# facebookresearch/PoseDiffusion

Measured on AMD Instinct MI355X. Metric: sequences/sec (20-frame, GGS on), higher is better.
Workload: dtype f32 (GGS, attention, LayerNorm, DDPM update, every accumulation); the encoder GEMMs multiply fp16 hi + lo operand pairs (22 bits, static power-of-two scales) with fp32 accumulation -- `exact_mode` is the same pipe with them on the exact-fp32 matrix instruction

## Files before the change

### posediffusion_amd/csrc/pd_qkv_attn.h

```cpp
#pragma once
#include "pd_gemm_split.h"

#ifndef PD_QA_XCD_MAP
#define PD_QA_XCD_MAP 1
#endif
#define PD_QA_WAVES 12
#define PD_QA_THREADS (PD_QA_WAVES * 64)
#define PD_QA_ROWS 96
#define PD_QA_LDR (3 * DH + 4)
#define PD_QA_LS 36
#ifndef PD_QA_DEEP_DEFAULT
#define PD_QA_DEEP_DEFAULT 0
#endif

struct PdQkvAttnArgs {
    const unsigned *A;
    const unsigned *W;
    const float *bias;
    unsigned *ctx;
    int B, N, G;
    float c_scale, out_scale;
};
static inline int pd_qkv_attn_group(int N) { return N >= 1 && N <= 32 ? (PD_QA_ROWS - 1) / N : 0; }
static inline int pd_qkv_attn_wgs(int B, int N) {
    const int G = pd_qkv_attn_group(N);
    return G ? ((B + G - 1) / G) * NH : 0;
}
static inline size_t pd_qkv_attn_lds(int N) {
    const int G = pd_qkv_attn_group(N);
    const size_t image = (size_t)(G * N + 1) * PD_QA_LDR * sizeof(float);
    const size_t stage = (size_t)4 * PD_QA_ROWS * 32 * sizeof(unsigned);
    return (image > stage ? image : stage) + (size_t)3 * 32 * PD_QA_LS * sizeof(float);
}

template <int BARE, bool DEEP = false>
__global__ __launch_bounds__(PD_QA_THREADS) void pd_qkv_attn_kernel(PdQkvAttnArgs g) {
    constexpr int KC = 32, RT = 3, TM = PD_QA_ROWS, CHA = TM * KC, LDR = PD_QA_LDR, LS = PD_QA_LS;
    constexpr bool M16 = PD_STRIP_MFMA16 != 0;
    extern __shared__ __attribute__((aligned(1024))) unsigned qa_lds[];
    const int tid = threadIdx.x, lane = tid & 63, l31 = lane & 31, hi = lane >> 5;
    const int wave = __builtin_amdgcn_readfirstlane(tid >> 6);
    int head = blockIdx.x & 3, grp = blockIdx.x >> 2;
#if PD_QA_XCD_MAP == 1
    {
        const int ngrp = gridDim.x >> 2, c = blockIdx.x >> 4, r = blockIdx.x & 15;
        if (4 * c + 4 <= ngrp) {
            head = 2 * ((r & 7) >> 2) + (r >> 3);
            grp = 4 * c + (r & 3);
        }
    }
#elif PD_QA_XCD_MAP == 2
    {
        const int ngrp = gridDim.x >> 2, c = blockIdx.x >> 5, r = blockIdx.x & 31;
        if (8 * c + 8 <= ngrp) {
            head = r >> 3;
            grp = 8 * c + (r & 7);
        }
    }
#endif
    const int N = g.N, G = g.G, M = g.B * N;
    const int seq0 = grp * G, nseq = min(G, g.B - seq0), m0 = seq0 * N, rows = nseq * N;
    const int nt16 = __builtin_amdgcn_readfirstlane((rows + 15) >> 4);
    const int stages = __builtin_amdgcn_readfirstlane(8 * wave < 16 * nt16 ? 1 : 0);
    const int prow = lane >> 3, pslot = lane & 7, l15 = lane & 15, kg = lane >> 4;
    unsigned oa;
    {
        const int r = 8 * wave + prow;
        oa = (unsigned)(((size_t)min(m0 + r, M - 1) * DM + 4 * (pslot ^ pd_strip_swz<M16>(r))) * sizeof(unsigned));
    }
    const unsigned lds_a = (unsigned)(size_t)(qa_lds + wave * 256);
    const int third = wave >> 2;
    const int ntile = third * (DM / 32) + head * (DH / 32) + (wave & 3);
    constexpr int KS = DM / 16;
    const uint4 *wq = (const uint4 *)g.W + (size_t)ntile * KS * 128 + (M16 ? (kg >> 1) * 128 + (kg & 1) * 32 + l15 : lane);
    typedef unsigned wv4 __attribute__((ext_vector_type(4)));
    f32x16 acc[M16 ? 1 : RT];
    f32x4 acc4[M16 ? 2 * RT : 1][2];
#pragma unroll
    for (int mi = 0; mi < (M16 ? 1 : RT); ++mi)
#pragma unroll
        for (int i = 0; i < 16; ++i) acc[mi][i] = 0.0f;
#pragma unroll
    for (int t = 0; t < (M16 ? 2 * RT : 1); ++t) acc4[t][0] = acc4[t][1] = f32x4{0.f, 0.f, 0.f, 0.f};
    auto mmaw = [](const uint4 &a, const wv4 &b, const f32x16 &c) {
        return __builtin_amdgcn_mfma_f32_32x32x16_f16(__builtin_bit_cast(f16x8, a), __builtin_bit_cast(f16x8, b), c, 0, 0, 0);
    };
    auto mma16 = [](const uint4 &a, const wv4 &b, const f32x4 &c) {
        return __builtin_amdgcn_mfma_f32_16x16x32_f16(__builtin_bit_cast(f16x8, a), __builtin_bit_cast(f16x8, b), c, 0, 0, 0);
    };
#define PD_QA_WLOAD(w0, w1, w2, w3, b)                                                                                               \
    do {                                                                                                                             \
        const uint4 *wp_ = wq + (size_t)(b) * 256;                                                                                   \
        if constexpr (M16)                                                                                                           \
            asm volatile("global_load_dwordx4 %0, %4, off\n\tglobal_load_dwordx4 %1, %4, off offset:1024\n\t"                       \
                         "global_load_dwordx4 %2, %4, off offset:256\n\tglobal_load_dwordx4 %3, %4, off offset:1280"                 \
                         : "=&v"(w0), "=&v"(w1), "=&v"(w2), "=&v"(w3) : "v"(wp_) : "memory");                                        \
        else                                                                                                                         \
            asm volatile("global_load_dwordx4 %0, %4, off\n\tglobal_load_dwordx4 %1, %4, off offset:1024\n\t"                       \
                         "global_load_dwordx4 %2, %4, off offset:2048\n\tglobal_load_dwordx4 %3, %4, off offset:3072"                \
                         : "=&v"(w0), "=&v"(w1), "=&v"(w2), "=&v"(w3) : "v"(wp_) : "memory");                                        \
    } while (0)
#define PD_QA_WAIT(n, w0, w1, w2, w3) asm volatile("s_waitcnt vmcnt(" #n ")" : "+v"(w0), "+v"(w1), "+v"(w2), "+v"(w3) : : "memory")
#define PD_QA_WAIT_STAGED(stg, w0, w1, w2, w3)                                                                                       \
    asm volatile("s_cmp_eq_u32 %4, 0\n\ts_cbranch_scc1 .Lqa_ns%=\n\ts_waitcnt vmcnt(6)\n\ts_branch .Lqa_done%=\n"                   \
                 ".Lqa_ns%=:\n\ts_waitcnt vmcnt(4)\n.Lqa_done%=:"                                                                   \
                 : "+v"(w0), "+v"(w1), "+v"(w2), "+v"(w3) : "s"(__builtin_amdgcn_readfirstlane(stg)) : "memory", "scc")
    auto stage64 = [&](int c, int buf) {
        if (!stages) return;
        const unsigned da = __builtin_amdgcn_readfirstlane(lds_a + buf * 2 * CHA * 4);
#pragma unroll
        for (int h = 0; h < 2; ++h) pd_dma_piece((const float *)(g.A + (2 * c + h) * KC), oa, da + h * CHA * 4);
    };
    auto block = [&](auto nt_, const unsigned *a, const wv4 &w0, const wv4 &w1, const wv4 &w2, const wv4 &w3) {
        constexpr int NT = decltype(nt_)::value;
        if constexpr (M16) {
            const int sz = pd_strip_swz<true>(l15);
#pragma unroll
            for (int t = 0; t < NT; ++t) {
                const uint4 p = *(const uint4 *)(a + t * 16 * KC + 4 * ((2 * kg) ^ sz));
                const uint4 q = *(const uint4 *)(a + t * 16 * KC + 4 * ((2 * kg + 1) ^ sz));
                const uint4 h8 = make_uint4(__builtin_amdgcn_perm(p.y, p.x, 0x05040100u), __builtin_amdgcn_perm(p.w, p.z, 0x05040100u),
                                            __builtin_amdgcn_perm(q.y, q.x, 0x05040100u), __builtin_amdgcn_perm(q.w, q.z, 0x05040100u));
                const uint4 l8 = make_uint4(__builtin_amdgcn_perm(p.y, p.x, 0x07060302u), __builtin_amdgcn_perm(p.w, p.z, 0x07060302u),
                                            __builtin_amdgcn_perm(q.y, q.x, 0x07060302u), __builtin_amdgcn_perm(q.w, q.z, 0x07060302u));
                f32x4 &c0 = acc4[M16 ? t : 0][0], &c1 = acc4[M16 ? t : 0][1];
                c0 = mma16(l8, w0, c0); c1 = mma16(l8, w2, c1);
                c0 = mma16(h8, w1, c0); c1 = mma16(h8, w3, c1);
                c0 = mma16(h8, w0, c0); c1 = mma16(h8, w2, c1);
            }
        } else {
        uint4 ah[RT], al[RT];
#pragma unroll
        for (int st = 0; st < 2; ++st) {
#pragma unroll
            for (int mi = 0; mi < RT; ++mi) {
                const uint4 p = *(const uint4 *)(a + mi * 32 * KC + 4 * ((4 * st + 2 * hi) ^ ((l31 >> 1) & 7)));
                const uint4 q = *(const uint4 *)(a + mi * 32 * KC + 4 * ((4 * st + 2 * hi + 1) ^ ((l31 >> 1) & 7)));
                ah[mi] = make_uint4(__builtin_amdgcn_perm(p.y, p.x, 0x05040100u), __builtin_amdgcn_perm(p.w, p.z, 0x05040100u),
                                    __builtin_amdgcn_perm(q.y, q.x, 0x05040100u), __builtin_amdgcn_perm(q.w, q.z, 0x05040100u));
                al[mi] = make_uint4(__builtin_amdgcn_perm(p.y, p.x, 0x07060302u), __builtin_amdgcn_perm(p.w, p.z, 0x07060302u),
                                    __builtin_amdgcn_perm(q.y, q.x, 0x07060302u), __builtin_amdgcn_perm(q.w, q.z, 0x07060302u));
            }
            const wv4 &wh = st ? w2 : w0, &wl = st ? w3 : w1;
#pragma unroll
            for (int mi = 0; mi < RT; ++mi) acc[M16 ? 0 : mi] = mmaw(al[mi], wh, acc[M16 ? 0 : mi]);
#pragma unroll
            for (int mi = 0; mi < RT; ++mi) acc[M16 ? 0 : mi] = mmaw(ah[mi], wl, acc[M16 ? 0 : mi]);
#pragma unroll
            for (int mi = 0; mi < RT; ++mi) acc[M16 ? 0 : mi] = mmaw(ah[mi], wh, acc[M16 ? 0 : mi]);
        }
        }
    };
    const int lrow = M16 ? l15 : l31;
    auto kloop = [&](auto nt_) {
        wv4 a0, a1, a2, a3, b0, b1, b2, b3;
        constexpr int nk64 = DM / 64;
        stage64(0, 0);
        PD_QA_WLOAD(a0, a1, a2, a3, 0);
        PD_QA_WLOAD(b0, b1, b2, b3, 1);
        PD_QA_WAIT(0, a0, a1, a2, a3);
        PD_QA_WAIT(0, b0, b1, b2, b3);
        __syncthreads();
        if constexpr (DEEP) {
            static_assert(!DEEP || BARE == 0, "the deep form has no development variants");
            wv4 c0, c1, c2, c3, d0, d1, d2, d3;
            for (int c = 0; c < nk64; c += 2) {
                {
                    const unsigned *a = qa_lds + 0 * 2 * CHA + lrow * KC;
                    stage64(c + 1, 1);
                    PD_QA_WLOAD(c0, c1, c2, c3, 2 * (c + 1));
                    PD_QA_WLOAD(d0, d1, d2, d3, 2 * (c + 1) + 1);
                    block(nt_, a, a0, a1, a2, a3);
                    block(nt_, a + CHA, b0, b1, b2, b3);
                    PD_QA_WAIT(0, c0, c1, c2, c3);
                    PD_QA_WAIT(0, d0, d1, d2, d3);
                    __syncthreads();
                }
                {
                    const int cn = min(c + 2, nk64 - 1);
                    const unsigned *a = qa_lds + 1 * 2 * CHA + lrow * KC;
                    stage64(cn, 0);
                    PD_QA_WLOAD(a0, a1, a2, a3, 2 * cn);
                    PD_QA_WLOAD(b0, b1, b2, b3, 2 * cn + 1);
                    block(nt_, a, c0, c1, c2, c3);
                    block(nt_, a + CHA, d0, d1, d2, d3);
                    PD_QA_WAIT(0, a0, a1, a2, a3);
                    PD_QA_WAIT(0, b0, b1, b2, b3);
                    __syncthreads();
                }
            }
        } else
        for (int c = 0; c < nk64; ++c) {
            const int cn = min(c + 1, nk64 - 1);
            const unsigned *a = qa_lds + (c & 1) * 2 * CHA + lrow * KC;
            if constexpr (BARE == 0) {
                if (c + 1 < nk64) {
                    stage64(cn, (c + 1) & 1);
                    block(nt_, a, a0, a1, a2, a3);
                    PD_QA_WLOAD(a0, a1, a2, a3, 2 * cn);
                    PD_QA_WAIT_STAGED(stages, b0, b1, b2, b3);
                    block(nt_, a + CHA, b0, b1, b2, b3);
                    PD_QA_WLOAD(b0, b1, b2, b3, 2 * cn + 1);
                    PD_QA_WAIT(4, a0, a1, a2, a3);
                } else {
                    block(nt_, a, a0, a1, a2, a3);
                    PD_QA_WAIT(0, b0, b1, b2, b3);
                    block(nt_, a + CHA, b0, b1, b2, b3);
                }
            } else {
                if constexpr (BARE != 2 && BARE != 3) stage64(cn, (c + 1) & 1);
                if constexpr (BARE != 4) block(nt_, a, a0, a1, a2, a3);
                if constexpr (BARE != 1 && BARE != 3) PD_QA_WLOAD(a0, a1, a2, a3, 2 * cn);
                if constexpr (BARE != 4) block(nt_, a + CHA, b0, b1, b2, b3);
                if constexpr (BARE != 1 && BARE != 3) PD_QA_WLOAD(b0, b1, b2, b3, 2 * cn + 1);
                PD_QA_WAIT(0, a0, a1, a2, a3);
                PD_QA_WAIT(0, b0, b1, b2, b3);
            }
            __syncthreads();
        }
        PD_QA_WAIT(0, b0, b1, b2, b3);
    };
    if constexpr (M16) {
        switch (nt16) {
        case 1: kloop(std::integral_constant<int, 1>()); break;
        case 2: kloop(std::integral_constant<int, 2>()); break;
        case 3: kloop(std::integral_constant<int, 3>()); break;
        case 4: kloop(std::integral_constant<int, 4>()); break;
        case 5: kloop(std::integral_constant<int, 5>()); break;
        default: kloop(std::integral_constant<int, 6>()); break;
        }
    } else {
        kloop(std::integral_constant<int, 6>());
    }
#undef PD_QA_WLOAD
#undef PD_QA_WAIT
#undef PD_QA_WAIT_STAGED
    if constexpr (BARE == 5) {
        if (acc[0][0] + acc4[0][0][0] == 123.456f) g.ctx[tid] = 1u;
        return;
    }
    float *img = (float *)qa_lds;
    float *Sall = img + (size_t)(G * N + 1) * LDR;
    {
        const float qscale = 0.08838834764831845f;
        if constexpr (M16) {
#pragma unroll
            for (int ct = 0; ct < 2; ++ct) {
                const float bias = g.bias[ntile * 32 + 16 * ct + l15];
                const int lcol = third * DH + (wave & 3) * 32 + 16 * ct + l15;
#pragma unroll
                for (int t = 0; t < 2 * RT; ++t)
#pragma unroll
                    for (int i = 0; i < 4; ++i) {
                        const int row = 16 * t + 4 * kg + i;
                        float v = fmaf(acc4[M16 ? t : 0][ct][i], g.c_scale, bias);
                        if (third == 0) v *= qscale;
                        if (row < rows) img[row * LDR + lcol] = v;
                    }
            }
        } else {
        const int col = ntile * 32 + l31;
        const float bias = g.bias[col];
        const int lcol = third * DH + (wave & 3) * 32 + l31;
#pragma unroll
        for (int mi = 0; mi < RT; ++mi)
#pragma unroll
            for (int i = 0; i < 16; ++i) {
                const int row = mi * 32 + 4 * hi + (i & 3) + 8 * (i >> 2);
                float v = fmaf(acc[M16 ? 0 : mi][i], g.c_scale, bias);
                if (third == 0) v *= qscale;
                if (row < rows) img[row * LDR + lcol] = v;
            }
        }
        for (int c = tid; c < LDR; c += PD_QA_THREADS) img[G * N * LDR + c] = 0.0f;
    }
    __syncthreads();
    const int team = wave >> 2, tw = wave & 3, ttid = tid & 255;
    float *S = Sall + team * 32 * LS;
    const int rounds = (G + 2) / 3;
    for (int rd = 0; rd < rounds; ++rd) {
        const int s = rd * 3 + team;
        const bool active = s < nseq;
        const float *base = img + (size_t)s * N * LDR;
        const float *zrow = img + (size_t)G * N * LDR;
        auto rowp = [&](int j) { return j < N ? base + j * LDR : zrow; };
        if (active) {
            const float *qa = rowp(16 * (tw >> 1) + (lane & 15)) + 4 * (lane >> 4);
            const float *kb = rowp(16 * (tw & 1) + (lane & 15)) + DH + 4 * (lane >> 4);
            f32x4 sc = {0.f, 0.f, 0.f, 0.f};
#pragma unroll
            for (int c = 0; c < DH / 16; ++c) {
                const float4 a = *(const float4 *)(qa + 16 * c), k = *(const float4 *)(kb + 16 * c);
                sc = __builtin_amdgcn_mfma_f32_16x16x4f32(a.x, k.x, sc, 0, 0, 0);
                sc = __builtin_amdgcn_mfma_f32_16x16x4f32(a.y, k.y, sc, 0, 0, 0);
                sc = __builtin_amdgcn_mfma_f32_16x16x4f32(a.z, k.z, sc, 0, 0, 0);
                sc = __builtin_amdgcn_mfma_f32_16x16x4f32(a.w, k.w, sc, 0, 0, 0);
            }
            const int j = 16 * (tw & 1) + (lane & 15);
#pragma unroll
            for (int e = 0; e < 4; ++e) S[(16 * (tw >> 1) + 4 * (lane >> 4) + e) * LS + j] = sc[e];
        }
        __syncthreads();
        if (active) {
            const int i = ttid >> 3, sub = ttid & 7;
            float4 sv = *(const float4 *)(S + i * LS + 4 * sub);
            const int j0 = 4 * sub;
            sv.x = j0 + 0 < N ? sv.x : -INFINITY;
            sv.y = j0 + 1 < N ? sv.y : -INFINITY;
            sv.z = j0 + 2 < N ? sv.z : -INFINITY;
            sv.w = j0 + 3 < N ? sv.w : -INFINITY;
            float mx = fmaxf(fmaxf(sv.x, sv.y), fmaxf(sv.z, sv.w));
            mx = fmaxf(mx, __shfl_xor(mx, 1, 64));
            mx = fmaxf(mx, __shfl_xor(mx, 2, 64));
            mx = fmaxf(mx, __shfl_xor(mx, 4, 64));
            float4 e;
            e.x = j0 + 0 < N ? expf(sv.x - mx) : 0.0f;
            e.y = j0 + 1 < N ? expf(sv.y - mx) : 0.0f;
            e.z = j0 + 2 < N ? expf(sv.z - mx) : 0.0f;
            e.w = j0 + 3 < N ? expf(sv.w - mx) : 0.0f;
            const float inv = 1.0f / pd_sum8((e.x + e.y) + (e.z + e.w));
            e.x *= inv; e.y *= inv; e.z *= inv; e.w *= inv;
            *(float4 *)(S + i * LS + 4 * sub) = e;
        }
        __syncthreads();
        if (active) {
            f32x4 o[2][2];
#pragma unroll
            for (int rt = 0; rt < 2; ++rt)
#pragma unroll
                for (int ct = 0; ct < 2; ++ct) o[rt][ct] = f32x4{0.f, 0.f, 0.f, 0.f};
            const float *pa = S + (lane & 15) * LS + 4 * (lane >> 4);
            const int vcol = 2 * DH + 32 * tw + (lane & 15);
            const int jg = 4 * (lane >> 4);
#pragma unroll
            for (int c = 0; c < 2; ++c) {
                const float4 p0 = *(const float4 *)(pa + 16 * c), p1 = *(const float4 *)(pa + 16 * LS + 16 * c);
                float v0[4], v1[4];
#pragma unroll
                for (int e = 0; e < 4; ++e) {
                    const float *vr = rowp(16 * c + jg + e) + vcol;
                    v0[e] = vr[0];
                    v1[e] = vr[16];
                }
                const float a0[4] = {p0.x, p0.y, p0.z, p0.w}, a1[4] = {p1.x, p1.y, p1.z, p1.w};
#pragma unroll
                for (int e = 0; e < 4; ++e) {
                    o[0][0] = __builtin_amdgcn_mfma_f32_16x16x4f32(a0[e], v0[e], o[0][0], 0, 0, 0);
                    o[0][1] = __builtin_amdgcn_mfma_f32_16x16x4f32(a0[e], v1[e], o[0][1], 0, 0, 0);
                    o[1][0] = __builtin_amdgcn_mfma_f32_16x16x4f32(a1[e], v0[e], o[1][0], 0, 0, 0);
                    o[1][1] = __builtin_amdgcn_mfma_f32_16x16x4f32(a1[e], v1[e], o[1][1], 0, 0, 0);
                }
            }
#pragma unroll
            for (int rt = 0; rt < 2; ++rt)
#pragma unroll
                for (int e = 0; e < 4; ++e) {
                    const int i = 16 * rt + 4 * (lane >> 4) + e;
                    if (i < N) {
                        unsigned *out = g.ctx + (size_t)((seq0 + s) * N + i) * DM + head * DH + 32 * tw + (lane & 15);
#pragma unroll
                        for (int ct = 0; ct < 2; ++ct) out[16 * ct] = pd_split_word_as<2>(o[rt][ct][e], g.out_scale);
                    }
                }
        }
        __syncthreads();
    }
}

static inline void pd_qkv_attn(const unsigned *hn, const unsigned *Wh, const float *bias, unsigned *ctx, int B, int N, float c_scale, float out_scale,
                               hipStream_t s) {
    PdQkvAttnArgs g{hn, Wh, bias, ctx, B, N, pd_qkv_attn_group(N), c_scale, out_scale};
    const dim3 grid(pd_qkv_attn_wgs(B, N)), blk(PD_QA_THREADS);
    const size_t lds = pd_qkv_attn_lds(N);
#ifdef PD_DEV_KNOBS
    static const int bare = pd_dev_knob("PD_QA_BARE", 0);
    static const int deep = pd_dev_knob("PD_QA_DEEP", PD_QA_DEEP_DEFAULT);
    if (bare == 0 && !deep) { hipLaunchKernelGGL((pd_qkv_attn_kernel<0, false>), grid, blk, lds, s, g); return; }
    switch (bare) {
    case 1: hipLaunchKernelGGL(pd_qkv_attn_kernel<1>, grid, blk, lds, s, g); return;
    case 2: hipLaunchKernelGGL(pd_qkv_attn_kernel<2>, grid, blk, lds, s, g); return;
    case 3: hipLaunchKernelGGL(pd_qkv_attn_kernel<3>, grid, blk, lds, s, g); return;
    case 4: hipLaunchKernelGGL(pd_qkv_attn_kernel<4>, grid, blk, lds, s, g); return;
    case 5: hipLaunchKernelGGL(pd_qkv_attn_kernel<5>, grid, blk, lds, s, g); return;
    default: break;
    }
#endif
    hipLaunchKernelGGL((pd_qkv_attn_kernel<0, PD_QA_DEEP_DEFAULT != 0>), grid, blk, lds, s, g);
}
```

Baseline: 1105.

## Give each wave its own attention row tile and replace block barriers with wave syncs

The attention phase of the fused QKV+attention kernel no longer runs in rounds of three 4-wave teams separated by block-wide barriers. Each wave now owns one (sequence, 16-row) unit. It computes the scores for all 32 keys, does the softmax, and does the full 128-wide PV product, using only wavefront fences and barriers. The score scratch grows to hold every sequence's rows at once. Dropping the __syncthreads rounds should remove barrier stalls, but with 20 frames some of the 12 waves sit idle, and each wave carries more accumulators, which raises register pressure.

```diff
diff --git a/posediffusion_amd/csrc/pd_qkv_attn.h b/posediffusion_amd/csrc/pd_qkv_attn.h
--- a/posediffusion_amd/csrc/pd_qkv_attn.h
+++ b/posediffusion_amd/csrc/pd_qkv_attn.h
@@ -30,7 +30,7 @@
     const int G = pd_qkv_attn_group(N);
     const size_t image = (size_t)(G * N + 1) * PD_QA_LDR * sizeof(float);
     const size_t stage = (size_t)4 * PD_QA_ROWS * 32 * sizeof(unsigned);
-    return (image > stage ? image : stage) + (size_t)3 * 32 * PD_QA_LS * sizeof(float);
+    return (image > stage ? image : stage) + (size_t)PD_QA_ROWS * PD_QA_LS * sizeof(float);
 }
 
 template <int BARE, bool DEEP = false>
@@ -275,35 +275,48 @@
         for (int c = tid; c < LDR; c += PD_QA_THREADS) img[G * N * LDR + c] = 0.0f;
     }
     __syncthreads();
-    const int team = wave >> 2, tw = wave & 3, ttid = tid & 255;
-    float *S = Sall + team * 32 * LS;
-    const int rounds = (G + 2) / 3;
-    for (int rd = 0; rd < rounds; ++rd) {
-        const int s = rd * 3 + team;
-        const bool active = s < nseq;
+    float *S = Sall;
+    const float *zrow = img + (size_t)G * N * LDR;
+    const int nrt = (N + 15) >> 4, units = nseq * nrt;
+    auto wave_sync = [] {
+        __builtin_amdgcn_fence(__ATOMIC_SEQ_CST, "wavefront");
+        __builtin_amdgcn_wave_barrier();
+    };
+    for (int u = wave; u < units; u += PD_QA_WAVES) {
+        const int s = nrt == 2 ? u >> 1 : u, rt = nrt == 2 ? u & 1 : 0;
         const float *base = img + (size_t)s * N * LDR;
-        const float *zrow = img + (size_t)G * N * LDR;
         auto rowp = [&](int j) { return j < N ? base + j * LDR : zrow; };
-        if (active) {
-            const float *qa = rowp(16 * (tw >> 1) + (lane & 15)) + 4 * (lane >> 4);
-            const float *kb = rowp(16 * (tw & 1) + (lane & 15)) + DH + 4 * (lane >> 4);
-            f32x4 sc = {0.f, 0.f, 0.f, 0.f};
+        float *St = S + (size_t)(s * N + 16 * rt) * LS;
+        {
+            const float *qa = rowp(16 * rt + l15) + 4 * kg;
+            const float *kb0 = rowp(l15) + DH + 4 * kg, *kb1 = rowp(16 + l15) + DH + 4 * kg;
+            f32x4 sc0 = {0.f, 0.f, 0.f, 0.f}, sc1 = {0.f, 0.f, 0.f, 0.f};
 #pragma unroll
             for (int c = 0; c < DH / 16; ++c) {
-                const float4 a = *(const float4 *)(qa + 16 * c), k = *(const float4 *)(kb + 16 * c);
-                sc = __builtin_amdgcn_mfma_f32_16x16x4f32(a.x, k.x, sc, 0, 0, 0);
-                sc = __builtin_amdgcn_mfma_f32_16x16x4f32(a.y, k.y, sc, 0, 0, 0);
-                sc = __builtin_amdgcn_mfma_f32_16x16x4f32(a.z, k.z, sc, 0, 0, 0);
-                sc = __builtin_amdgcn_mfma_f32_16x16x4f32(a.w, k.w, sc, 0, 0, 0);
-            }
-            const int j = 16 * (tw & 1) + (lane & 15);
-#pragma unroll
-            for (int e = 0; e < 4; ++e) S[(16 * (tw >> 1) + 4 * (lane >> 4) + e) * LS + j] = sc[e];
-        }
-        __syncthreads();
-        if (active) {
-            const int i = ttid >> 3, sub = ttid & 7;
-            float4 sv = *(const float4 *)(S + i * LS + 4 * sub);
+                const float4 a = *(const float4 *)(qa + 16 * c), k0 = *(const float4 *)(kb0 + 16 * c), k1 = *(const float4 *)(kb1 + 16 * c);
+                sc0 = __builtin_amdgcn_mfma_f32_16x16x4f32(a.x, k0.x, sc0, 0, 0, 0);
+                sc1 = __builtin_amdgcn_mfma_f32_16x16x4f32(a.x, k1.x, sc1, 0, 0, 0);
+                sc0 = __builtin_amdgcn_mfma_f32_16x16x4f32(a.y, k0.y, sc0, 0, 0, 0);
+                sc1 = __builtin_amdgcn_mfma_f32_16x16x4f32(a.y, k1.y, sc1, 0, 0, 0);
+                sc0 = __builtin_amdgcn_mfma_f32_16x16x4f32(a.z, k0.z, sc0, 0, 0, 0);
+                sc1 = __builtin_amdgcn_mfma_f32_16x16x4f32(a.z, k1.z, sc1, 0, 0, 0);
+                sc0 = __builtin_amdgcn_mfma_f32_16x16x4f32(a.w, k0.w, sc0, 0, 0, 0);
+                sc1 = __builtin_amdgcn_mfma_f32_16x16x4f32(a.w, k1.w, sc1, 0, 0, 0);
+            }
+#pragma unroll
+            for (int e = 0; e < 4; ++e)
+                if (16 * rt + 4 * kg + e < N) {
+                    St[(4 * kg + e) * LS + l15] = sc0[e];
+                    St[(4 * kg + e) * LS + 16 + l15] = sc1[e];
+                }
+        }
+        wave_sync();
+#pragma unroll
+        for (int p = 0; p < 2; ++p) {
+            const int i = 8 * p + (lane >> 3), sub = lane & 7;
+            const bool live = 16 * rt + i < N;
+            float *sp = St + (live ? i : N - 1 - 16 * rt) * LS + 4 * sub;
+            float4 sv = *(const float4 *)sp;
             const int j0 = 4 * sub;
             sv.x = j0 + 0 < N ? sv.x : -INFINITY;
             sv.y = j0 + 1 < N ? sv.y : -INFINITY;
@@ -320,50 +333,40 @@
             e.w = j0 + 3 < N ? expf(sv.w - mx) : 0.0f;
             const float inv = 1.0f / pd_sum8((e.x + e.y) + (e.z + e.w));
             e.x *= inv; e.y *= inv; e.z *= inv; e.w *= inv;
-            *(float4 *)(S + i * LS + 4 * sub) = e;
-        }
-        __syncthreads();
-        if (active) {
-            f32x4 o[2][2];
-#pragma unroll
-            for (int rt = 0; rt < 2; ++rt)
-#pragma unroll
-                for (int ct = 0; ct < 2; ++ct) o[rt][ct] = f32x4{0.f, 0.f, 0.f, 0.f};
-            const float *pa = S + (lane & 15) * LS + 4 * (lane >> 4);
-            const int vcol = 2 * DH + 32 * tw + (lane & 15);
-            const int jg = 4 * (lane >> 4);
+            wave_sync();
+            if (live) *(float4 *)sp = e;
+        }
+        wave_sync();
+        {
+            f32x4 o[8];
+#pragma unroll
+            for (int ct = 0; ct < 8; ++ct) o[ct] = f32x4{0.f, 0.f, 0.f, 0.f};
+            const float *pa = St + min(l15, N - 1 - 16 * rt) * LS + 4 * kg;
+            const int vcol = 2 * DH + l15;
 #pragma unroll
             for (int c = 0; c < 2; ++c) {
-                const float4 p0 = *(const float4 *)(pa + 16 * c), p1 = *(const float4 *)(pa + 16 * LS + 16 * c);
-                float v0[4], v1[4];
+                const float4 p0 = *(const float4 *)(pa + 16 * c);
+                const float a0[4] = {p0.x, p0.y, p0.z, p0.w};
 #pragma unroll
                 for (int e = 0; e < 4; ++e) {
-                    const float *vr = rowp(16 * c + jg + e) + vcol;
-                    v0[e] = vr[0];
-                    v1[e] = vr[16];
-                }
-                const float a0[4] = {p0.x, p0.y, p0.z, p0.w}, a1[4] = {p1.x, p1.y, p1.z, p1.w};
-#pragma unroll
-                for (int e = 0; e < 4; ++e) {
-                    o[0][0] = __builtin_amdgcn_mfma_f32_16x16x4f32(a0[e], v0[e], o[0][0], 0, 0, 0);
-                    o[0][1] = __builtin_amdgcn_mfma_f32_16x16x4f32(a0[e], v1[e], o[0][1], 0, 0, 0);
-                    o[1][0] = __builtin_amdgcn_mfma_f32_16x16x4f32(a1[e], v0[e], o[1][0], 0, 0, 0);
-                    o[1][1] = __builtin_amdgcn_mfma_f32_16x16x4f32(a1[e], v1[e], o[1][1], 0, 0, 0);
-                }
-            }
-#pragma unroll
-            for (int rt = 0; rt < 2; ++rt)
-#pragma unroll
-                for (int e = 0; e < 4; ++e) {
-                    const int i = 16 * rt + 4 * (lane >> 4) + e;
-                    if (i < N) {
-                        unsigned *out = g.ctx + (size_t)((seq0 + s) * N + i) * DM + head * DH + 32 * tw + (lane & 15);
-#pragma unroll
-                        for (int ct = 0; ct < 2; ++ct) out[16 * ct] = pd_split_word_as<2>(o[rt][ct][e], g.out_scale);
-                    }
-                }
-        }
-        __syncthreads();
+                    const float *vr = rowp(16 * c + 4 * kg + e) + vcol;
+                    float v[8];
+#pragma unroll
+                    for (int ct = 0; ct < 8; ++ct) v[ct] = vr[16 * ct];
+#pragma unroll
+                    for (int ct = 0; ct < 8; ++ct) o[ct] = __builtin_amdgcn_mfma_f32_16x16x4f32(a0[e], v[ct], o[ct], 0, 0, 0);
+                }
+            }
+#pragma unroll
+            for (int e = 0; e < 4; ++e) {
+                const int i = 16 * rt + 4 * kg + e;
+                if (i < N) {
+                    unsigned *out = g.ctx + (size_t)((seq0 + s) * N + i) * DM + head * DH + l15;
+#pragma unroll
+                    for (int ct = 0; ct < 8; ++ct) out[16 * ct] = pd_split_word_as<2>(o[ct][e], g.out_scale);
+                }
+            }
+        }
     }
 }
 
```

Measured after the change: 1111, median of 6. Within noise of the previous version (+0.5%).
